# RainbowXXX/3DReconstruction

Measured on AMD Instinct MI355X. Metric: BA LM-iters/sec + obs/sec, 1k cams/500k pts/5M obs; SIFT match pairs/sec, higher is better.
Workload: dtype f64; 1 GPU; C4 BA 1000 cams / 500000 pts / 5000000 obs, banded orbit visibility k=10, HuberLoss(4), gauge image 1, Ceres-default LM to termination per step; parallelism=landmark-sharded x1, all-reduce of the RCS, transport=none

## Files before the change

### 3dreconstruction_amd/csrc/ba_schur.hip

```cpp
#include "ba_device.h"
namespace sfm {
namespace {

struct alignas(16) CamPreL {
    CamPre cp;
    double pad[2];
};
template <int SP = kSubPts, int SO = kSubObs>
__device__ __forceinline__ int batch_points(const int* cpoff, int p0, int np) {
    const int lane = threadIdx.x & 63, q1 = p0 + 1 + lane;
    const bool fits = lane < SP && q1 <= np && cpoff[q1] - cpoff[p0] <= SO;
    return __builtin_ctzll(~__ballot(fits));
}

__device__ constexpr int kTi[15] = {0, 1, 1, 2, 2, 2, 3, 3, 3, 3, 4, 4, 4, 4, 4};
__device__ constexpr int kTj[15] = {0, 0, 1, 0, 1, 2, 0, 1, 2, 3, 0, 1, 2, 3, 4};

template <int CM, int NT, int SP = kSubPts, int SO = kSubObs, bool SE = false>
__global__ __launch_bounds__(64 * schur_group(NT)) __attribute__((amdgpu_waves_per_eu(2, 2))) void schur_kernel(
    DevProblem P, const CamPre* __restrict__ cps, const double* __restrict__ intr,
    const double* __restrict__ X, double radius, unsigned long long* __restrict__ stamps) {
    constexpr int IW = kIW<CM>;
    constexpr int NK = CM == SFM_CAM_SNAVELY ? 3 : IW;
    unsigned long long tacc[6] = {0, 0, 0, 0, 0, 0}, tprev = 0;
    if (stamps) tprev = stamp();
#define SFM_STAMP(k)                                      \
    if (stamps) {                                         \
        const unsigned long long tn_ = stamp();           \
        tacc[k] += tn_ - tprev;                           \
        tprev = tn_;                                      \
    }
    constexpr int kPK = 4 * ((3 * SP + 3) / 4), kPR = 16 * NT, kPS = kPR + 4;
    constexpr int kOb = CM == SFM_CAM_PINHOLE ? 5 : 2 * NK + 1;
    constexpr int kNTiles = NT * (NT + 1) / 2;
    constexpr int kComb = 5;
    struct WaveLds {
        double panel[kPK][kPS];
        double wcol[NT == 4 ? kPK : 1];
        double ob[SO][kOb];
        double vs[SO][9];
        double vsum[SP][10];
        int orow[SO];
        int cpoff[kChunkPts + 1];
    };
    union WaveU {
        WaveLds w;
        double comb[kComb * 256 + 64];
    };
    static_assert(sizeof(WaveLds) >= sizeof(double) * (kComb * 256 + 64), "tile hand-over space");
    constexpr int GW = schur_group(NT);
    __shared__ WaveU wl[GW];
    __shared__ CamPreL scp[kCamSlots];
    __shared__ double csc[kCamSlots][6];
    __shared__ double isc[kIntrSlots][2 * IW];
    __shared__ int crow[kCamSlots], irow[kIntrSlots];
    const int wave = __builtin_amdgcn_readfirstlane(threadIdx.x >> 6), lane = threadIdx.x & 63, grp = blockIdx.x;
    const int c0 = P.group_off[grp], n_sub = P.group_off[grp + 1] - c0;
    const int c = c0 + (wave < n_sub ? wave : 0);
    const ChunkDesc& cd = P.chunks[c];
    WaveLds& W = wl[wave].w;
    double (&panel)[kPK][kPS] = W.panel;
    double (&wcol)[NT == 4 ? kPK : 1] = W.wcol;
    double (&ob)[SO][kOb] = W.ob;
    double (&vs)[SO][9] = W.vs;
    double (&vsum)[SP][10] = W.vsum;
    double (*const obm)[9] = vs;
    int (&orow)[SO] = W.orow;
    int (&cpoff)[kChunkPts + 1] = W.cpoff;
    const int pb = cd.pt_begin, np = wave < n_sub ? cd.pt_end - pb : 0, ob0 = cd.obs_begin;
    const bool one_intr = cd.n_intr == 1;
    const double inv_radius = 1.0 / radius;

    for (int e = lane; e <= np; e += 64) cpoff[e] = P.pt_off[pb + e] - ob0;
    {
        constexpr int kCpW = sizeof(CamPre) / 8;
        for (int e = threadIdx.x; e < cd.n_cams * kCpW; e += 64 * GW) {
            const int t = e / kCpW;
            reinterpret_cast<double*>(&scp[t].cp)[e - t * kCpW] =
                reinterpret_cast<const double*>(&cps[cd.cam_img[t]])[e - t * kCpW];
        }
        for (int e = threadIdx.x; e < cd.n_cams * 6; e += 64 * GW) {
            const int t = e / 6, col = cd.cam_col[t];
            csc[t][e - 6 * t] = col >= 0 ? P.scaleF[col + e - 6 * t] : 0.0;
        }
        if (threadIdx.x < cd.n_cams) crow[threadIdx.x] = cd.cam_row[threadIdx.x];
        if (threadIdx.x < IW * cd.n_intr) {
            const int t = threadIdx.x / IW, k = threadIdx.x - IW * t;
            isc[t][k] = intr[IW * cd.intr_id[t] + k];
            isc[t][IW + k] = P.scaleF[cd.intr_col[t] + k];
        }
        if (threadIdx.x < cd.n_intr) irow[threadIdx.x] = cd.intr_row[threadIdx.x];
    }

    v4d acc[kNTiles];
#pragma unroll
    for (int q = 0; q < kNTiles; ++q) acc[q] = v4d{0.0, 0.0, 0.0, 0.0};
    double wacc = 0.0;

    double xn2 = 0.0, gmx = 0.0;
    __syncthreads();
    struct BatchIn {
        int npts, slot, pl;
        double u0, u1, Xp[3], sE[3];
    };
    auto fetch = [&](int q0, BatchIn& in) {
        in.npts = q0 < np ? batch_points<SP, SO>(cpoff, q0, np) : 0;
        in.slot = 0; in.pl = 0; in.u0 = 0.0; in.u1 = 0.0;
#pragma unroll
        for (int k = 0; k < 3; ++k) { in.Xp[k] = 0.0; in.sE[k] = 1.0; }
        const int qo = cpoff[q0 < np ? q0 : np];
        if (lane < cpoff[q0 + in.npts] - qo) {
            const int o = ob0 + qo + lane;
            in.slot = P.obs_slot[o];
            const double2 uv = reinterpret_cast<const double2*>(P.obs_uv)[o];
            in.u0 = uv.x; in.u1 = uv.y;
#pragma unroll
            for (int j = 1; j < SP; ++j) in.pl += (j < in.npts && cpoff[q0 + j] - qo <= lane) ? 1 : 0;
            const size_t g = 3 * (size_t)(pb + q0 + in.pl);
#pragma unroll
            for (int k = 0; k < 3; ++k) { in.Xp[k] = X[g + k]; in.sE[k] = P.scaleE[g + k]; }
        }
    };
    BatchIn nx;
    fetch(0, nx);
    __builtin_amdgcn_s_waitcnt(0x0F70);
    for (int p0 = 0; p0 < np;) {
        const int npts = nx.npts;
        if (npts == 0) break;
        const int p1 = p0 + npts;
        const int o0 = cpoff[p0], nobs = cpoff[p1] - o0;
        const int slot = nx.slot, pl = nx.pl;
        const double u0 = nx.u0, u1 = nx.u1;
        const double Xp[3] = {nx.Xp[0], nx.Xp[1], nx.Xp[2]};
        double sE[3] = {nx.sE[0], nx.sE[1], nx.sE[2]};
        fetch(p1, nx);
#pragma unroll
        for (int e = lane; e < kPK * kPS / 2; e += 64)
            reinterpret_cast<double2*>(&panel[0][0])[e] = double2{0.0, 0.0};
        if constexpr (NT == 4)
            if (lane < kPK) wcol[lane] = 0.0;
        SFM_STAMP(0)
        LinT<CM> L;
        const int cs = slot & 255, is = (slot >> 8) & 255;
        if (lane < nobs) linearize<CM, true, true, true>(scp[cs].cp, &isc[is][0], Xp, u0, u1, P.huber_a, L);
        if constexpr (SE) {
            if (lane < nobs) {
#pragma unroll
                for (int r = 0; r < 2; ++r)
#pragma unroll
                    for (int a = 0; a < 3; ++a) obm[lane][3 * r + a] = L.Jx[r][a];
            }
            wsync();
            if (lane < 3 * npts) {
                const int pt = lane / 3, a = lane - 3 * pt;
                const int q0 = cpoff[p0 + pt] - o0, q1 = cpoff[p0 + pt + 1] - o0;
                double cn = 0.0;
                for (int q = q0; q < q1; ++q) {
                    cn = fma(obm[q][a], obm[q][a], cn);
                    cn = fma(obm[q][3 + a], obm[q][3 + a], cn);
                }
                const double se = 1.0 / (1.0 + sqrt(cn));
                vsum[pt][a] = se;
                P.scaleE[3 * (size_t)(pb + p0 + pt) + a] = se;
            }
            wsync();
            if (lane < nobs) {
#pragma unroll
                for (int a = 0; a < 3; ++a) sE[a] = vsum[pl][a];
            }
            wsync();
        }
        if (lane < nobs) {
#pragma unroll
            for (int r = 0; r < 2; ++r) {
#pragma unroll
                for (int a = 0; a < 6; ++a) L.Jc[r][a] *= csc[cs][a];
#pragma unroll
                for (int a = 0; a < 3; ++a) L.Jx[r][a] *= sE[a];
            }
            double cv[9] = {0, 0, 0, 0, 0, 0, 0, 0, 0};
#pragma unroll
            for (int r = 0; r < 2; ++r) {
                const double j0 = L.Jx[r][0], j1 = L.Jx[r][1], j2 = L.Jx[r][2], fr = L.f[r];
                cv[0] += j0 * j0; cv[1] += j1 * j0; cv[2] += j1 * j1;
                cv[3] += j2 * j0; cv[4] += j2 * j1; cv[5] += j2 * j2;
                cv[6] += j0 * fr; cv[7] += j1 * fr; cv[8] += j2 * fr;
            }
#pragma unroll
            for (int e = 0; e < 9; ++e) vs[lane][e] = cv[e];
            if constexpr (CM != SFM_CAM_PINHOLE) {
#pragma unroll
                for (int k = 0; k < NK; ++k) {
                    ob[lane][2 * k] = L.Ji[0][k] * isc[is][IW + k];
                    ob[lane][2 * k + 1] = L.Ji[1][k] * isc[is][IW + k];
                }
            } else {
                ob[lane][0] = L.Ji[0][0] * isc[is][4];
                ob[lane][1] = L.Ji[1][1] * isc[is][5];
                ob[lane][2] = L.Ji[0][2] * isc[is][6];
                ob[lane][3] = L.Ji[1][3] * isc[is][7];
            }
            orow[lane] = irow[is];
        }
        wsync();
        if (lane < 9 * npts) {
            const int pt = lane / 9, e = lane - 9 * pt;
            const int q0 = cpoff[p0 + pt] - o0, q1 = cpoff[p0 + pt + 1] - o0;
            double acc = 0.0;
            int q = q0;
            for (; q + 4 <= q1; q += 4) {
                const double v0 = vs[q][e], v1 = vs[q + 1][e], v2 = vs[q + 2][e], v3 = vs[q + 3][e];
                acc += v0; acc += v1; acc += v2; acc += v3;
            }
            for (; q < q1; ++q) acc += vs[q][e];
            vsum[pt][e] = acc;
        }
        wsync();
        SFM_STAMP(1)
        if (lane < nobs) {
            const int q0 = cpoff[p0 + pl] - o0;
            double V[6], b[3];
#pragma unroll
            for (int e = 0; e < 6; ++e) V[e] = vsum[pl][e];
#pragma unroll
            for (int e = 0; e < 3; ++e) b[e] = vsum[pl][6 + e];
            const bool first = lane == q0;
            if (first) {
#pragma unroll
                for (int a = 0; a < 3; ++a) {
                    const double g = b[a] * rcp_nr(sE[a]);
                    xn2 += Xp[a] * Xp[a];
                    gmx = fmax(gmx, fabs(Xp[a] - (Xp[a] - g)));
                }
            }
            const auto [i00, i10, i11, i20, i21, i22] = point_factor(P, V, inv_radius);
            if (first) {
                const double w3[3] = {i00 * b[0], i10 * b[0] + i11 * b[1], i20 * b[0] + i21 * b[1] + i22 * b[2]};
#pragma unroll
                for (int a = 0; a < 3; ++a) {
                    if constexpr (NT == 5) panel[3 * pl + a][kTileWRow % kPR] = w3[a];
                    else wcol[3 * pl + a] = w3[a];
                }
            }
            double M[2][3];
#pragma unroll
            for (int r = 0; r < 2; ++r) {
                M[r][0] = L.Jx[r][0] * i00;
                M[r][1] = L.Jx[r][0] * i10 + L.Jx[r][1] * i11;
                M[r][2] = L.Jx[r][0] * i20 + L.Jx[r][1] * i21 + L.Jx[r][2] * i22;
            }
            const int row = crow[cs];
            if (row >= 0) {
#pragma unroll
                for (int a = 0; a < 3; ++a)
#pragma unroll
                    for (int k = 0; k < 6; ++k)
                        panel[3 * pl + a][row + k] = L.Jc[0][k] * M[0][a] + L.Jc[1][k] * M[1][a];
            }
#pragma unroll
            for (int r = 0; r < 2; ++r)
#pragma unroll
                for (int a = 0; a < 3; ++a) obm[lane][3 * r + a] = M[r][a];
        }
        wsync();
        SFM_STAMP(2)
        if (one_intr) {
            constexpr int NZ = 3 * NK;
            const int row = irow[0];
            for (int e = lane; e < NZ * npts; e += 64) {
                const int pt = e / NZ, rem = e - NZ * pt, a = rem / NK, k = rem - NK * a;
                const int q0 = cpoff[p0 + pt] - o0, q1 = cpoff[p0 + pt + 1] - o0;
                double z = 0.0;
                int q = q0;
                if constexpr (CM == SFM_CAM_PINHOLE) {
                    const int mo = 3 * (k & 1) + a;
                    for (; q + 4 <= q1; q += 4) {
                        double jv[4], mv[4];
#pragma unroll
                        for (int j = 0; j < 4; ++j) { jv[j] = ob[q + j][k]; mv[j] = obm[q + j][mo]; }
#pragma unroll
                        for (int j = 0; j < 4; ++j) z = fma(jv[j], mv[j], z);
                    }
                    for (; q < q1; ++q) z = fma(ob[q][k], obm[q][mo], z);
                } else {
                    for (; q + 2 <= q1; q += 2) {
                        double jv[4], mv[4];
#pragma unroll
                        for (int j = 0; j < 2; ++j) {
                            jv[2 * j] = ob[q + j][2 * k]; jv[2 * j + 1] = ob[q + j][2 * k + 1];
                            mv[2 * j] = obm[q + j][a]; mv[2 * j + 1] = obm[q + j][3 + a];
                        }
#pragma unroll
                        for (int j = 0; j < 4; ++j) z = fma(jv[j], mv[j], z);
                    }
                    for (; q < q1; ++q) {
                        z = fma(ob[q][2 * k], obm[q][a], z);
                        z = fma(ob[q][2 * k + 1], obm[q][3 + a], z);
                    }
                }
                panel[3 * pt + a][row + k] += z;
            }
        } else if constexpr (CM != SFM_CAM_PINHOLE) {
            for (int e = lane; e < 3 * NK * npts; e += 64) {
                const int pt = e / (3 * NK), rem = e - 3 * NK * pt, a = rem / NK, k = rem - NK * a;
                const int q0 = cpoff[p0 + pt] - o0, q1 = cpoff[p0 + pt + 1] - o0;
                int row = orow[q0];
                double z = 0.0;
                for (int q = q0; q < q1; ++q) {
                    const int rq = orow[q];
                    if (rq != row) {
                        panel[3 * pt + a][row + k] += z;
                        z = 0.0;
                        row = rq;
                    }
                    z = fma(ob[q][2 * k], obm[q][a], z);
                    z = fma(ob[q][2 * k + 1], obm[q][3 + a], z);
                }
                panel[3 * pt + a][row + k] += z;
            }
        } else if constexpr (12 * SP <= 64) {
            if (lane < 12 * npts) {
                const int pt = lane / 12, rem = lane - 12 * pt, a = rem >> 2, k = rem & 3;
                const int mo = 3 * (k & 1) + a;
                const int q0 = cpoff[p0 + pt] - o0, q1 = cpoff[p0 + pt + 1] - o0;
                int row = orow[q0];
                double z = 0.0;
                auto step = [&](int rq, double jv, double mv) {
                    if (rq != row) {
                        panel[3 * pt + a][row + k] += z;
                        z = 0.0;
                        row = rq;
                    }
                    z = fma(jv, mv, z);
                };
                int q = q0;
                for (; q + 4 <= q1; q += 4) {
                    int rq[4];
                    double jv[4], mv[4];
#pragma unroll
                    for (int j = 0; j < 4; ++j) { rq[j] = orow[q + j]; jv[j] = ob[q + j][k]; mv[j] = obm[q + j][mo]; }
#pragma unroll
                    for (int j = 0; j < 4; ++j) step(rq[j], jv[j], mv[j]);
                }
                for (; q < q1; ++q) step(orow[q], ob[q][k], obm[q][mo]);
                panel[3 * pt + a][row + k] += z;
            }
        } else if (lane < 3 * npts) {
            const int pt = lane / 3, a = lane - 3 * pt;
            const int q0 = cpoff[p0 + pt] - o0, q1 = cpoff[p0 + pt + 1] - o0;
            int row = orow[q0];
            double z0 = 0.0, z1 = 0.0, z2 = 0.0, z3 = 0.0;
            for (int q = q0; q < q1; ++q) {
                const int rq = orow[q];
                if (rq != row) {
                    panel[3 * pt + a][row + 0] += z0; panel[3 * pt + a][row + 1] += z1;
                    panel[3 * pt + a][row + 2] += z2; panel[3 * pt + a][row + 3] += z3;
                    z0 = z1 = z2 = z3 = 0.0;
                    row = rq;
                }
                const double m0 = obm[q][a], m1 = obm[q][3 + a];
                z0 += ob[q][0] * m0;
                z1 += ob[q][1] * m1;
                z2 += ob[q][2] * m0;
                z3 += ob[q][3] * m1;
            }
            panel[3 * pt + a][row + 0] += z0; panel[3 * pt + a][row + 1] += z1;
            panel[3 * pt + a][row + 2] += z2; panel[3 * pt + a][row + 3] += z3;
        }
        wsync();
        SFM_STAMP(3)
        const int kk = lane >> 4, ii = lane & 15;
        constexpr int kKs = kPK / 4;
        double op[kKs][NT];
#pragma unroll
        for (int ks = 0; ks < kKs; ++ks)
#pragma unroll
            for (int t = 0; t < NT; ++t) op[ks][t] = panel[4 * ks + kk][16 * t + ii];
#pragma unroll
        for (int ks = 0; ks < kKs; ++ks)
#pragma unroll
            for (int q = 0; q < kNTiles; ++q)
                acc[q] = __builtin_amdgcn_mfma_f64_16x16x4f64(op[ks][kTi[q]], op[ks][kTj[q]], acc[q], 0, 0, 0);
        if constexpr (NT == 4) {
#pragma unroll
            for (int k = 0; k < kPK; ++k) wacc += panel[k][lane] * wcol[k];
        }
        wsync();
        SFM_STAMP(4)
        p0 = p1;
    }
    __syncthreads();
    double* out = P.tiles + (size_t)grp * kTileR * kTileR;
#pragma unroll
    for (int q0 = 0; q0 < kNTiles; q0 += kComb) {
        if (wave > 0 && wave < n_sub) {
            double* cb = wl[wave].comb;
#pragma unroll
            for (int q = q0; q < q0 + kComb && q < kNTiles; ++q)
#pragma unroll
                for (int r = 0; r < 4; ++r) cb[(q - q0) * 256 + r * 64 + lane] = acc[q][r];
            if (NT == 4 && q0 == 0) cb[kComb * 256 + lane] = wacc;
        }
        __syncthreads();
        if (wave == 0) {
            for (int w2 = 1; w2 < n_sub; ++w2) {
                const double* cb = wl[w2].comb;
#pragma unroll
                for (int q = q0; q < q0 + kComb && q < kNTiles; ++q)
#pragma unroll
                    for (int r = 0; r < 4; ++r) acc[q][r] += cb[(q - q0) * 256 + r * 64 + lane];
                if (NT == 4 && q0 == 0) wacc += cb[kComb * 256 + lane];
            }
#pragma unroll
            for (int q = q0; q < q0 + kComb && q < kNTiles; ++q) {
                const int ti = kTi[q], tj = kTj[q];
#pragma unroll
                for (int r = 0; r < 4; ++r) {
                    const int row = 16 * ti + (lane >> 4) + 4 * r, col = 16 * tj + (lane & 15);
                    out[row * kTileR + col] = -acc[q][r];
                }
            }
            if (NT == 4 && q0 == 0) out[kTileWRow * kTileR + lane] = -wacc;
        }
        if (q0 + kComb < kNTiles) __syncthreads();
    }
    double s1[1] = {xn2};
    wave_sum(s1);
    const double m1 = wave_max(gmx);
    if (lane == 0 && wave < n_sub) {
        P.part_s[2 * (size_t)c] = s1[0];
        P.part_s[2 * (size_t)c + 1] = m1;
    }
    SFM_STAMP(5)
    if (stamps && lane == 0 && wave < n_sub)
        for (int k = 0; k < 6; ++k) stamps[6 * (size_t)c + k] = tacc[k];
#undef SFM_STAMP
}


constexpr int kZStage = 19;

template <int CM, bool SE>
__global__ __launch_bounds__(64) void zpoint_kernel(DevProblem P, const CamPre* __restrict__ cps,
                                                    const double* __restrict__ intr, const double* __restrict__ X,
                                                    double radius) {
    extern __shared__ __attribute__((aligned(16))) double zlds[];
    double* zc = zlds;
    double* Zl = zlds + 64 * kZStage;
    __shared__ int cbl[64];
    const int lane = threadIdx.x, g = P.zlong[blockIdx.x];
    const int k = P.n_cpt + g;
    const int o0 = P.pt_off[k], o1 = P.pt_off[k + 1];
    const int b0 = P.gblk_off[g];
    const int zn = (int)(P.gz_off[g + 1] - P.gz_off[g]) - 3;
    const double Xp[3] = {X[3 * (size_t)k], X[3 * (size_t)k + 1], X[3 * (size_t)k + 2]};
    double sE[3];
    constexpr int IW = kIW<CM>;
    auto lin = [&](int o, LinT<CM>& L) {
        const int img = P.obs_img[o];
        const double2 uv = reinterpret_cast<const double2*>(P.obs_uv)[o];
        linearize<CM, true, true, true>(cps[img], intr + IW * (size_t)P.img_intr[img], Xp, uv.x, uv.y, P.huber_a, L);
    };
    if constexpr (SE) {
        double cn[3] = {0.0, 0.0, 0.0};
        for (int o = o0 + lane; o < o1; o += 64) {
            LinT<CM> L;
            lin(o, L);
#pragma unroll
            for (int a = 0; a < 3; ++a) cn[a] += L.Jx[0][a] * L.Jx[0][a] + L.Jx[1][a] * L.Jx[1][a];
        }
        wave_sum(cn);
#pragma unroll
        for (int a = 0; a < 3; ++a) sE[a] = 1.0 / (1.0 + sqrt(cn[a]));
        if (lane < 3) P.scaleE[3 * (size_t)k + lane] = sE[lane];
    } else {
#pragma unroll
        for (int a = 0; a < 3; ++a) sE[a] = P.scaleE[3 * (size_t)k + a];
    }
    double v9[9] = {0, 0, 0, 0, 0, 0, 0, 0, 0};
    for (int o = o0 + lane; o < o1; o += 64) {
        LinT<CM> L;
        lin(o, L);
#pragma unroll
        for (int r = 0; r < 2; ++r) {
            const double j0 = L.Jx[r][0] * sE[0], j1 = L.Jx[r][1] * sE[1], j2 = L.Jx[r][2] * sE[2], fr = L.f[r];
            v9[0] += j0 * j0; v9[1] += j1 * j0; v9[2] += j1 * j1;
            v9[3] += j2 * j0; v9[4] += j2 * j1; v9[5] += j2 * j2;
            v9[6] += j0 * fr; v9[7] += j1 * fr; v9[8] += j2 * fr;
        }
    }
    wave_sum(v9);
    double V[6] = {v9[0], v9[1], v9[2], v9[3], v9[4], v9[5]};
    const double b[3] = {v9[6], v9[7], v9[8]};
    if (lane == 0) {
        double xn2 = 0.0, gmx = 0.0;
        point_norms(b, sE, Xp, xn2, gmx);
        P.part_s[2 * (size_t)(P.n_chunk + g)] = xn2;
        P.part_s[2 * (size_t)(P.n_chunk + g) + 1] = gmx;
    }
    const auto [i00, i10, i11, i20, i21, i22] = point_factor(P, V, 1.0 / radius);
    for (int e = lane; e < zn; e += 64) Zl[e] = 0.0;
    int prev_cb = -1;
    for (int base = o0; base < o1; base += 64) {
        const int o = base + lane;
        const bool act = o < o1;
        int cb = 0xffff, ib = -1;
        double zi[3 * IW];
#pragma unroll
        for (int e = 0; e < 3 * IW; ++e) zi[e] = 0.0;
        if (act) {
            LinT<CM> L;
            lin(o, L);
            const int img = P.obs_img[o];
            const int slot = P.obs_slot[o];
            cb = slot & 0xffff;
            ib = slot >> 16;
            double M[2][3];
#pragma unroll
            for (int r = 0; r < 2; ++r) {
                const double j0 = L.Jx[r][0] * sE[0], j1 = L.Jx[r][1] * sE[1], j2 = L.Jx[r][2] * sE[2];
                M[r][0] = j0 * i00;
                M[r][1] = j0 * i10 + j1 * i11;
                M[r][2] = j0 * i20 + j1 * i21 + j2 * i22;
            }
            const int colc = P.img_colc[img], coli = P.img_coli[img];
            if (cb != 0xffff) {
#pragma unroll
                for (int r = 0; r < 6; ++r) {
                    const double s = P.scaleF[colc + r];
#pragma unroll
                    for (int a = 0; a < 3; ++a)
                        zc[lane * kZStage + 3 * r + a] = (L.Jc[0][r] * s) * M[0][a] + (L.Jc[1][r] * s) * M[1][a];
                }
            }
            const int ni = CM == SFM_CAM_SNAVELY ? 3 : IW;
#pragma unroll
            for (int r = 0; r < IW; ++r) {
                if (r >= ni) continue;
                const double s = P.scaleF[coli + r];
#pragma unroll
                for (int a = 0; a < 3; ++a) zi[3 * r + a] = (L.Ji[0][r] * s) * M[0][a] + (L.Ji[1][r] * s) * M[1][a];
            }
        }
        cbl[lane] = act ? cb : -2;
        wsync();
        const bool head = act && cb != 0xffff && (lane == 0 || cbl[lane - 1] != cb);
        if (head) {
            double acc[18];
#pragma unroll
            for (int e = 0; e < 18; ++e) acc[e] = zc[lane * kZStage + e];
            for (int q = lane + 1; q < 64 && cbl[q] == cb; ++q)
#pragma unroll
                for (int e = 0; e < 18; ++e) acc[e] += zc[q * kZStage + e];
            double* dst = Zl + P.gblk_z[b0 + cb];
            const bool cont = lane == 0 && cb == prev_cb;
#pragma unroll
            for (int e = 0; e < 18; ++e) dst[e] = cont ? dst[e] + acc[e] : acc[e];
        }
        prev_cb = cbl[63] >= 0 ? cbl[63] : -1;
        unsigned long long pend = __ballot(act);
        while (pend) {
            const int src = __builtin_ctzll(pend);
            const int j = __shfl(ib, src);
            const bool mine = act && ib == j;
            double v[3 * IW];
#pragma unroll
            for (int e = 0; e < 3 * IW; ++e) v[e] = mine ? zi[e] : 0.0;
            wave_sum(v);
            const int nz = 3 * (CM == SFM_CAM_SNAVELY ? 3 : IW);
            double mine_v = 0.0;
#pragma unroll
            for (int e = 0; e < 3 * IW; ++e) mine_v = lane == e ? v[e] : mine_v;
            if (lane < nz) Zl[P.gblk_z[b0 + j] + lane] += mine_v;
            pend &= ~__ballot(mine);
        }
        wsync();
    }
    double* Zg = P.Z + P.gz_off[g];
    for (int e = lane; e < zn; e += 64) Zg[e] = Zl[e];
    if (lane < 3) {
        const double w3[3] = {i00 * b[0], i10 * b[0] + i11 * b[1], i20 * b[0] + i21 * b[1] + i22 * b[2]};
        Zg[zn + lane] = lane == 0 ? w3[0] : lane == 1 ? w3[1] : w3[2];
    }
}

constexpr int kZRow = 19;
template <int CM, bool SE>
__global__ __launch_bounds__(64) void zbatch_kernel(DevProblem P, const CamPre* __restrict__ cps,
                                                    const double* __restrict__ intr, const double* __restrict__ X,
                                                    double radius) {
    constexpr int IW = kIW<CM>;
    constexpr int NI = CM == SFM_CAM_SNAVELY ? 3 : IW;
    __shared__ double rc[64][kZRow];
    __shared__ double pv[kZBatchPts][12];
    __shared__ int poff[kZBatchPts + 1], okey[64], oib[64];
    const int lane = threadIdx.x;
    const int g0 = P.zbatch[2 * blockIdx.x], g1 = P.zbatch[2 * blockIdx.x + 1], np = g1 - g0;
    const int oA = P.pt_off[P.n_cpt + g0];
    if (lane <= np) poff[lane] = P.pt_off[P.n_cpt + g0 + lane] - oA;
    wsync();
    const int nobs = poff[np];
    const bool act = lane < nobs;
    int pl = 0;
    for (int j = 1; j < np; ++j) pl += poff[j] <= lane ? 1 : 0;
    const int g = g0 + pl, k = P.n_cpt + g, o = oA + lane;
    const bool head = act && lane == poff[pl];
    double Xp[3] = {0.0, 0.0, 0.0};
    LinT<CM> L{};
    int img = 0, cb = 0xffff, ib = 0;
    if (act) {
#pragma unroll
        for (int a = 0; a < 3; ++a) Xp[a] = X[3 * (size_t)k + a];
        img = P.obs_img[o];
        const int slot = P.obs_slot[o];
        cb = slot & 0xffff;
        ib = slot >> 16;
        const double2 uv = reinterpret_cast<const double2*>(P.obs_uv)[o];
        linearize<CM, true, true, true>(cps[img], intr + IW * (size_t)P.img_intr[img], Xp, uv.x, uv.y, P.huber_a, L);
    }
    auto point_sum = [&](int n, int at) {
        wsync();
        if (head) {
            for (int e = 0; e < n; ++e) {
                double acc = rc[lane][e];
                for (int q = lane + 1; q < poff[pl + 1]; ++q) acc += rc[q][e];
                pv[pl][at + e] = acc;
            }
        }
        wsync();
    };
    double sE[3];
    if constexpr (SE) {
        if (act)
#pragma unroll
            for (int a = 0; a < 3; ++a) rc[lane][a] = L.Jx[0][a] * L.Jx[0][a] + L.Jx[1][a] * L.Jx[1][a];
        point_sum(3, 9);
        if (head)
#pragma unroll
            for (int a = 0; a < 3; ++a) {
                const double se = 1.0 / (1.0 + sqrt(pv[pl][9 + a]));
                pv[pl][9 + a] = se;
                P.scaleE[3 * (size_t)k + a] = se;
            }
        wsync();
#pragma unroll
        for (int a = 0; a < 3; ++a) sE[a] = pv[pl][9 + a];
    } else {
#pragma unroll
        for (int a = 0; a < 3; ++a) sE[a] = act ? P.scaleE[3 * (size_t)k + a] : 1.0;
    }
    double j[2][3];
#pragma unroll
    for (int r = 0; r < 2; ++r)
#pragma unroll
        for (int a = 0; a < 3; ++a) j[r][a] = L.Jx[r][a] * sE[a];
    if (act) {
        double v9[9] = {0, 0, 0, 0, 0, 0, 0, 0, 0};
#pragma unroll
        for (int r = 0; r < 2; ++r) {
            const double fr = L.f[r];
            v9[0] += j[r][0] * j[r][0]; v9[1] += j[r][1] * j[r][0]; v9[2] += j[r][1] * j[r][1];
            v9[3] += j[r][2] * j[r][0]; v9[4] += j[r][2] * j[r][1]; v9[5] += j[r][2] * j[r][2];
            v9[6] += j[r][0] * fr; v9[7] += j[r][1] * fr; v9[8] += j[r][2] * fr;
        }
#pragma unroll
        for (int e = 0; e < 9; ++e) rc[lane][e] = v9[e];
    }
    point_sum(9, 0);
    double V[6], b[3];
#pragma unroll
    for (int e = 0; e < 6; ++e) V[e] = pv[pl][e];
#pragma unroll
    for (int e = 0; e < 3; ++e) b[e] = pv[pl][6 + e];
    if (head) {
        double xn2 = 0.0, gmx = 0.0;
        point_norms(b, sE, Xp, xn2, gmx);
        P.part_s[2 * (size_t)(P.n_chunk + g)] = xn2;
        P.part_s[2 * (size_t)(P.n_chunk + g) + 1] = gmx;
    }
    const auto [i00, i10, i11, i20, i21, i22] = point_factor(P, V, 1.0 / radius);
    double M[2][3];
#pragma unroll
    for (int r = 0; r < 2; ++r) {
        M[r][0] = j[r][0] * i00;
        M[r][1] = j[r][0] * i10 + j[r][1] * i11;
        M[r][2] = j[r][0] * i20 + j[r][1] * i21 + j[r][2] * i22;
    }
    if (act) {
        if (cb != 0xffff) {
            const int colc = P.img_colc[img];
#pragma unroll
            for (int r = 0; r < 6; ++r) {
                const double sc = P.scaleF[colc + r];
#pragma unroll
                for (int a = 0; a < 3; ++a) rc[lane][3 * r + a] = (L.Jc[0][r] * sc) * M[0][a] + (L.Jc[1][r] * sc) * M[1][a];
            }
        }
    }
    okey[lane] = act ? (pl << 17 | cb) : -1;
    oib[lane] = ib;
    wsync();
    double* Zp = P.Z + P.gz_off[g];
    const int b0 = P.gblk_off[g], pend = poff[pl + 1];
    if (act) {
        if (cb != 0xffff && (lane == poff[pl] || okey[lane - 1] != okey[lane])) {
            double acc[18];
#pragma unroll
            for (int e = 0; e < 18; ++e) acc[e] = rc[lane][e];
            for (int q = lane + 1; q < pend && okey[q] == okey[lane]; ++q)
#pragma unroll
                for (int e = 0; e < 18; ++e) acc[e] += rc[q][e];
            double* dst = Zp + P.gblk_z[b0 + cb];
#pragma unroll
            for (int e = 0; e < 18; ++e) dst[e] = acc[e];
        }
    }
    wsync();
    if (act) {
        const int coli = P.img_coli[img];
#pragma unroll
        for (int r = 0; r < NI; ++r) {
            const double sc = P.scaleF[coli + r];
#pragma unroll
            for (int a = 0; a < 3; ++a) rc[lane][3 * r + a] = (L.Ji[0][r] * sc) * M[0][a] + (L.Ji[1][r] * sc) * M[1][a];
        }
    }
    wsync();
    if (act) {
        bool first = true;
        for (int q = poff[pl]; q < lane; ++q) first = first && oib[q] != ib;
        if (first) {
            double acc[3 * NI];
#pragma unroll
            for (int e = 0; e < 3 * NI; ++e) acc[e] = rc[lane][e];
            for (int q = lane + 1; q < pend; ++q)
                if (oib[q] == ib)
#pragma unroll
                    for (int e = 0; e < 3 * NI; ++e) acc[e] += rc[q][e];
            double* dst = Zp + P.gblk_z[b0 + ib];
#pragma unroll
            for (int e = 0; e < 3 * IW; ++e) dst[e] = e < 3 * NI ? acc[e < 3 * NI ? e : 0] : 0.0;
        }
        if (head) {
            const int zn = (int)(P.gz_off[g + 1] - P.gz_off[g]) - 3;
            Zp[zn] = i00 * b[0];
            Zp[zn + 1] = i10 * b[0] + i11 * b[1];
            Zp[zn + 2] = i20 * b[0] + i21 * b[1] + i22 * b[2];
        }
    }
}

}

void ba_schur(const DevProblem& P, const CamPre* cp, const double* intr, const double* X, double radius,
              hipStream_t s, unsigned long long* stamps, bool scale_e) {
    by_flag(scale_e, [&](auto tag) {
        constexpr bool SE = decltype(tag)::value;
        if (P.n_zbatch > 0) {
            SFM_BY_MODEL_ALL(P, hipLaunchKernelGGL((zbatch_kernel<CM, SE>), dim3(P.n_zbatch), dim3(64), 0, s, P, cp,
                                                   intr, X, radius));
            SFM_HIP(hipGetLastError());
        }
        if (P.n_zlong > 0) {
            const size_t lds = (64 * kZStage + (size_t)P.gz_max) * sizeof(double);
            SFM_BY_MODEL_ALL(P, {
                if (lds > 64 * 1024) set_dyn_lds((const void*)zpoint_kernel<CM, SE>, lds);
                hipLaunchKernelGGL((zpoint_kernel<CM, SE>), dim3(P.n_zlong), dim3(64), lds, s, P, cp, intr, X, radius);
            });
            SFM_HIP(hipGetLastError());
        }
        if (P.n_group <= 0) return;
        const dim3 grid(P.n_group), block(64 * schur_group(P.tile_nt));
        if (P.tile_nt == 4)
            SFM_BY_MODEL_ALL(P, hipLaunchKernelGGL((schur_kernel<CM, 4, schur4_pts(CM), schur4_obs(CM), SE>), grid, block,
                                                   0, s, P, cp, intr, X, radius, stamps));
        else
            SFM_BY_MODEL_ALL(P, hipLaunchKernelGGL((schur_kernel<CM, 5, kSubPts, kSubObs, SE>), grid, block, 0, s, P, cp,
                                                   intr, X, radius, stamps));
        SFM_HIP(hipGetLastError());
    });
}

}
```

### 3dreconstruction_amd/csrc/ba_types.h

```cpp
#pragma once
#include <cstdint>

namespace sfm {

constexpr int kTileN = 5;
constexpr int kTileR = 16 * kTileN;
constexpr int kTileRowsUsed = 76;
constexpr int kTileWRow = 79;
constexpr int kSubPts = 6;
constexpr int kZShortObs = 32;
constexpr int kZBatchPts = 16;
constexpr int kSubObs = 64;
constexpr int schur4_pts(int cm) { return cm == 0 ? 5 : 4; }
constexpr int schur4_obs(int cm) { return cm == 0 ? 52 : cm == 2 ? 44 : 48; }
constexpr int kChunkPts = 128;
constexpr int kGroupChunks = 4;
constexpr int schur_group(int) { return 1; }
constexpr int kGramSeg = 3;
constexpr int kMaxSlots = 16;
constexpr int kCamSlots = 14;
constexpr int kIntrSlots = 4;
constexpr int kZMaxDoubles = 18432;

struct SourceLayout {
    int64_t fw, o_u, o_ub, o_ucn, n_total;
    SourceLayout(int64_t n_group, int64_t n_img, int32_t iw) : fw(6 + iw) {
        o_u = (n_group > 1 ? n_group : 1) * kTileR * kTileR;
        o_ub = o_u + fw * fw * n_img * kGramSeg;
        o_ucn = o_ub + fw * n_img * kGramSeg;
        n_total = o_ucn + fw * n_img * kGramSeg;
    }
};

struct alignas(16) CamPre {
    double c, s, omc, small;
    double u[3];
    double t[3];
    double R[9];
    double Ar[9];
};

struct ChunkDesc {
    int32_t pt_begin, pt_end;
    int32_t obs_begin, obs_end;
    int32_t n_slots;
    int32_t n_cams, n_intr;
    int32_t sub;
    int32_t cam_img[kCamSlots];
    int32_t cam_row[kCamSlots];
    int32_t cam_col[kCamSlots];
    int32_t intr_id[kIntrSlots];
    int32_t intr_row[kIntrSlots];
    int32_t intr_col[kIntrSlots];
    int32_t slot_img[kMaxSlots];
    int32_t slot_intr[kMaxSlots];
    int32_t slot_row[kMaxSlots];
    int32_t slot_col[kMaxSlots];
};

enum : int32_t { kSrcTile = 0, kSrcU = 1, kSrcUb = 2, kSrcUcn = 3 };

struct ReduceTarget {
    int64_t dst;
    int32_t dst_kind;
    int32_t rows, cols;
    int32_t ld;
    int32_t c_begin, c_end;
    int32_t p_begin, p_end;
};

struct PTerm {
    int32_t za, zb;
};

enum : int32_t { kDstBand = 0, kDstArrow = 1, kDstCorner = 2, kDstRhs = 3, kDstBF = 4, kDstCnF = 5,
                 kDstDense = 6 };

enum : int16_t { kFlatRows = 0, kFlatTrans = 1, kFlatSym = 2 };
struct FlatTerm {
    int64_t off;
    int16_t rs;
    int16_t mode;
    float sign;
};

struct ReduceTerm {
    int32_t kind;
    int32_t index;
    int16_t roff, coff;
    float sign;
};

}
```

Before: 1159 LM-iters/s.

## Slim LDS layout for pinhole NT=4 Schur kernel to fit larger point batches

For the pinhole camera with four tiles, the per-wave LDS struct gets a slimmer form. The vs scratch now shares space with the panel through a union, the Jacobian rows and products sit interleaved in one row array, and cpoff and orow shrink to 16-bit and 8-bit. This frees enough LDS to raise the pinhole batch from 5 points/52 obs to 6 points/60 obs, and a dedicated one-intrinsic Z-accumulation path is added. Because of the union, panel zeroing has to move after the vs reduction, which adds an extra wave sync. The MFMA operand load is also guarded for the shorter panel K dimension.

Result: faster. 1191 LM-iters/s, median of 6 (+2.7%).

```diff
diff --git a/3dreconstruction_amd/csrc/ba_schur.hip b/3dreconstruction_amd/csrc/ba_schur.hip
--- a/3dreconstruction_amd/csrc/ba_schur.hip
+++ b/3dreconstruction_amd/csrc/ba_schur.hip
@@ -1,3 +1,5 @@
+#include <type_traits>
+
 #include "ba_device.h"
 namespace sfm {
 namespace {
@@ -6,12 +8,17 @@
     CamPre cp;
     double pad[2];
 };
-template <int SP = kSubPts, int SO = kSubObs>
-__device__ __forceinline__ int batch_points(const int* cpoff, int p0, int np) {
-    const int lane = threadIdx.x & 63, q1 = p0 + 1 + lane;
-    const bool fits = lane < SP && q1 <= np && cpoff[q1] - cpoff[p0] <= SO;
-    return __builtin_ctzll(~__ballot(fits));
+template <int SP = kSubPts, int SO = kSubObs, class Off>
+__device__ __forceinline__ int batch_points(const Off* cpoff, int p0, int np) {
+    const int lane = threadIdx.x & 63;
+    return __builtin_ctzll(~__ballot(batch_fits(cpoff, p0, lane, np, SP, SO)));
 }
+
+template <int S>
+struct LdsRows {
+    double* p;
+    __device__ __forceinline__ double* operator[](int q) const { return p + q * S; }
+};
 
 __device__ constexpr int kTi[15] = {0, 1, 1, 2, 2, 2, 3, 3, 3, 3, 4, 4, 4, 4, 4};
 __device__ constexpr int kTj[15] = {0, 0, 1, 0, 1, 2, 0, 1, 2, 3, 0, 1, 2, 3, 4};
@@ -34,7 +41,11 @@
     constexpr int kOb = CM == SFM_CAM_PINHOLE ? 5 : 2 * NK + 1;
     constexpr int kNTiles = NT * (NT + 1) / 2;
     constexpr int kComb = 5;
-    struct WaveLds {
+    constexpr bool kSlim = NT == 4 && CM == SFM_CAM_PINHOLE;
+    constexpr int kPKs = kSlim ? 3 * SP : kPK;
+    constexpr int kObU = CM == SFM_CAM_PINHOLE ? 4 : 2 * NK;
+    constexpr int kRow = (kObU + 6) | 1;
+    struct WaveLdsWide {
         double panel[kPK][kPS];
         double wcol[NT == 4 ? kPK : 1];
         double ob[SO][kOb];
@@ -43,6 +54,20 @@
         int orow[SO];
         int cpoff[kChunkPts + 1];
     };
+    struct WaveLdsSlim {
+        union {
+            double panel[kPKs][kPS];
+            double vs[SO][9];
+        };
+        double wcol[kPKs];
+        double row[SO][kRow];
+        double vsum[SP][10];
+        unsigned short cpoff[kChunkPts + 1];
+        unsigned char orow[SO];
+    };
+    static_assert(!kSlim || (sizeof(double) * SO * 9 <= sizeof(double) * kPKs * kPS && kChunkPts * SO < 65536),
+                  "slim layout: the shares fit the panel, the offsets 16 bits");
+    using WaveLds = std::conditional_t<kSlim, WaveLdsSlim, WaveLdsWide>;
     union WaveU {
         WaveLds w;
         double comb[kComb * 256 + 64];
@@ -59,14 +84,21 @@
     const int c = c0 + (wave < n_sub ? wave : 0);
     const ChunkDesc& cd = P.chunks[c];
     WaveLds& W = wl[wave].w;
-    double (&panel)[kPK][kPS] = W.panel;
-    double (&wcol)[NT == 4 ? kPK : 1] = W.wcol;
-    double (&ob)[SO][kOb] = W.ob;
-    double (&vs)[SO][9] = W.vs;
+    double (&panel)[kPKs][kPS] = W.panel;
+    auto& wcol = W.wcol;
+    const LdsRows<9> vs{&W.vs[0][0]};
+    LdsRows<kSlim ? kRow : kOb> ob;
+    LdsRows<kSlim ? kRow : 9> obm;
+    if constexpr (kSlim) {
+        ob.p = &W.row[0][0];
+        obm.p = &W.row[0][kObU];
+    } else {
+        ob.p = &W.ob[0][0];
+        obm.p = &W.vs[0][0];
+    }
     double (&vsum)[SP][10] = W.vsum;
-    double (*const obm)[9] = vs;
-    int (&orow)[SO] = W.orow;
-    int (&cpoff)[kChunkPts + 1] = W.cpoff;
+    auto& orow = W.orow;
+    auto& cpoff = W.cpoff;
     const int pb = cd.pt_begin, np = wave < n_sub ? cd.pt_end - pb : 0, ob0 = cd.obs_begin;
     const bool one_intr = cd.n_intr == 1;
     const double inv_radius = 1.0 / radius;
@@ -134,11 +166,14 @@
         const double Xp[3] = {nx.Xp[0], nx.Xp[1], nx.Xp[2]};
         double sE[3] = {nx.sE[0], nx.sE[1], nx.sE[2]};
         fetch(p1, nx);
-#pragma unroll
-        for (int e = lane; e < kPK * kPS / 2; e += 64)
-            reinterpret_cast<double2*>(&panel[0][0])[e] = double2{0.0, 0.0};
-        if constexpr (NT == 4)
-            if (lane < kPK) wcol[lane] = 0.0;
+        auto zero_panel = [&]() {
+#pragma unroll
+            for (int e = lane; e < kPKs * kPS / 2; e += 64)
+                reinterpret_cast<double2*>(&panel[0][0])[e] = double2{0.0, 0.0};
+            if constexpr (NT == 4)
+                if (lane < kPKs) wcol[lane] = 0.0;
+        };
+        if constexpr (!kSlim) zero_panel();
         SFM_STAMP(0)
         LinT<CM> L;
         const int cs = slot & 255, is = (slot >> 8) & 255;
@@ -216,6 +251,10 @@
             vsum[pt][e] = acc;
         }
         wsync();
+        if constexpr (kSlim) {
+            zero_panel();
+            wsync();
+        }
         SFM_STAMP(1)
         if (lane < nobs) {
             const int q0 = cpoff[p0 + pl] - o0;
@@ -264,7 +303,26 @@
         }
         wsync();
         SFM_STAMP(2)
-        if (one_intr) {
+        if (kSlim && one_intr && 12 * SP > 64) {
+            const int row = irow[0];
+            if (lane < 6 * npts) {
+                const int pt = lane / 6, rem = lane - 6 * pt, a = rem >> 1, r = rem & 1;
+                const int mo = 3 * r + a;
+                const int q0 = cpoff[p0 + pt] - o0, q1 = cpoff[p0 + pt + 1] - o0;
+                double z0 = 0.0, z2 = 0.0;
+                int q = q0;
+                for (; q + 4 <= q1; q += 4) {
+                    double j0[4], j2[4], mv[4];
+#pragma unroll
+                    for (int j = 0; j < 4; ++j) { j0[j] = ob[q + j][r]; j2[j] = ob[q + j][r + 2]; mv[j] = obm[q + j][mo]; }
+#pragma unroll
+                    for (int j = 0; j < 4; ++j) { z0 = fma(j0[j], mv[j], z0); z2 = fma(j2[j], mv[j], z2); }
+                }
+                for (; q < q1; ++q) { z0 = fma(ob[q][r], obm[q][mo], z0); z2 = fma(ob[q][r + 2], obm[q][mo], z2); }
+                panel[3 * pt + a][row + r] += z0;
+                panel[3 * pt + a][row + r + 2] += z2;
+            }
+        } else if (one_intr) {
             constexpr int NZ = 3 * NK;
             const int row = irow[0];
             for (int e = lane; e < NZ * npts; e += 64) {
@@ -375,7 +433,8 @@
 #pragma unroll
         for (int ks = 0; ks < kKs; ++ks)
 #pragma unroll
-            for (int t = 0; t < NT; ++t) op[ks][t] = panel[4 * ks + kk][16 * t + ii];
+            for (int t = 0; t < NT; ++t)
+                op[ks][t] = (4 * ks + 3 < kPKs || 4 * ks + kk < kPKs) ? panel[4 * ks + kk][16 * t + ii] : 0.0;
 #pragma unroll
         for (int ks = 0; ks < kKs; ++ks)
 #pragma unroll
@@ -383,7 +442,7 @@
                 acc[q] = __builtin_amdgcn_mfma_f64_16x16x4f64(op[ks][kTi[q]], op[ks][kTj[q]], acc[q], 0, 0, 0);
         if constexpr (NT == 4) {
 #pragma unroll
-            for (int k = 0; k < kPK; ++k) wacc += panel[k][lane] * wcol[k];
+            for (int k = 0; k < kPKs; ++k) wacc += panel[k][lane] * wcol[k];
         }
         wsync();
         SFM_STAMP(4)
diff --git a/3dreconstruction_amd/csrc/ba_types.h b/3dreconstruction_amd/csrc/ba_types.h
--- a/3dreconstruction_amd/csrc/ba_types.h
+++ b/3dreconstruction_amd/csrc/ba_types.h
@@ -11,8 +11,18 @@
 constexpr int kZShortObs = 32;
 constexpr int kZBatchPts = 16;
 constexpr int kSubObs = 64;
-constexpr int schur4_pts(int cm) { return cm == 0 ? 5 : 4; }
-constexpr int schur4_obs(int cm) { return cm == 0 ? 52 : cm == 2 ? 44 : 48; }
+constexpr int schur4_pts(int cm) { return cm == 0 ? 6 : 4; }
+constexpr int schur4_obs(int cm) { return cm == 0 ? 60 : cm == 2 ? 44 : 48; }
+template <class Off>
+constexpr bool batch_fits(const Off* off, int p0, int j, int np, int sp, int so) {
+    return j < sp && p0 + 1 + j <= np && (int)off[p0 + 1 + j] - (int)off[p0] <= so;
+}
+template <class Off>
+constexpr int batch_count(const Off* off, int p0, int np, int sp, int so) {
+    int j = 0;
+    while (batch_fits(off, p0, j, np, sp, so)) ++j;
+    return j;
+}
 constexpr int kChunkPts = 128;
 constexpr int kGroupChunks = 4;
 constexpr int schur_group(int) { return 1; }
```
